# tarepan/DDSP-SVC-official

Hardware: AMD Instinct MI355X
Metric: audio samples/sec @44.1kHz CombSub synth (higher is better)
Workload: dtype f32 storage and accumulation; products of the GEMM / FIR contractions split-bf16x3 (hi*hi+hi*lo+lo*hi), of the attention split-bf16 from three pieces (6 products) for the feature projections and two (3 products) for the context sums; everything else f32; `value_fp32_mfma` is the leg with every produ; 1 GPU; CombSub 44.1 kHz, batch=64x2 s per GPU (Fr=172, T=88064), units/f0/volume/spk_id -> audio, seeded random weights, in-kernel noise

## Files before the change

ddsp-svc-official_amd/csrc/gemm_f32.h:

```cpp
#pragma once
#include "common.h"

#include <stdlib.h>
#include <type_traits>

namespace gemm {

enum { A_PLAIN = 0, A_CONV3 = 1, A_FRAMES = 2, A_CONVK = 3 };

struct Args {
    const float* A;
    const float* B;
    int M, N, K;
    int64_t lda, ldb;
    int zdiv;
    int64_t sA_hi, sA_lo, sB_hi, sB_lo;
    int Fr, Cin;
    int tap_shift;
    int ktaps, dil;
    float in_slope;
    const float* zeros;
    int sub_from, parent_tn;
    int math;
    const float* B_split;
    int A_split;
    int xcd;
    int xcd_cut;
    int kz;
};

constexpr int BK = 32;
// ... 800 lines not shown
```

ddsp-svc-official_amd/csrc/gemm_ln.h:

```cpp
#pragma once
#include "gemm_f32.h"

#include <atomic>
#include <stdlib.h>

namespace gemm {

struct LnArgs {
    const float* A;
    const float* W;
    int64_t lda, ldw;
    int M, K;
    const float* bias;
    const float* res;
    float* X;
    const float* gamma;
    const float* beta;
    float* Y;
    int y_split;
    int Fr = 1, Cin = 32, tap_shift = 0;
    const float* zeros = nullptr;
};

struct PreResidual {
    struct State {
        f32x4 res[2][4];
        f32x4 bias4[4];
    };
    template <int RB>
    __device__ __forceinline__ void load(State& s, const LnArgs& g, int m0, int rg0, int lr, int cg, int lh) const {
#pragma unroll
        for (int b = 0; b < RB; ++b) {
            const int row_m = m0 + 32 * (rg0 + b) + lr;
#pragma unroll
            for (int q = 0; q < 4; ++q) {
                s.res[b][q] = f32x4{0.f, 0.f, 0.f, 0.f};
                if (row_m < g.M) s.res[b][q] = *(const f32x4*)(g.res + (int64_t)row_m * 256 + 32 * cg + 8 * q + 4 * lh);
            }
        }
#pragma unroll
        for (int q = 0; q < 4; ++q) s.bias4[q] = *(const f32x4*)(g.bias + 32 * cg + 8 * q + 4 * lh);
    }
    __device__ __forceinline__ f32x4 apply(const State& s, const LnArgs&, int b, int q, int, int, f32x4 acc) const {
        f32x4 v;
#pragma unroll
        for (int e = 0; e < 4; ++e) v[e] = s.res[b][q][e] + (acc[e] + s.bias4[q][e]);
        return v;
    }
};

constexpr int LN_BM = 64, LN_N = 256, LN_NS = 4;
constexpr int LN_STAGE = (LN_BM + LN_N) * 32;
constexpr size_t LN_LDS_BYTES = (size_t)LN_NS * LN_STAGE * sizeof(float);

template <int NS, int RB, bool ASPLIT, int A_MODE, class Pre>
__global__ void __launch_bounds__(1024 / RB) kernel_res_ln(LnArgs g, Pre pre) {
    extern __shared__ __attribute__((aligned(1024))) float ln_lds[];
    float* const lds = ln_lds;
    constexpr int NWAVE = 16 / RB;
    const int tid = threadIdx.x, lane = tid & 63, wave = __builtin_amdgcn_readfirstlane(tid >> 6);
    const int rg0 = RB == 1 ? wave >> 3 : 0, cg = wave & 7, lr = lane & 31, lh = lane >> 5;
    const int nk = g.K / 32;
    const int m0 = blockIdx.x * LN_BM;

    typename Pre::State pst;
    pre.template load<RB>(pst, g, m0, rg0, lr, cg, lh);
    f32x4 gam4[4], bet4[4];
#pragma unroll
    for (int q = 0; q < 4; ++q) {
        const int c0 = 32 * cg + 8 * q + 4 * lh;
        gam4[q] = *(const f32x4*)(g.gamma + c0);
        bet4[q] = *(const f32x4*)(g.beta + c0);
    }

    constexpr int MAXP = RB == 1 ? 3 : 5;
    const float* src[MAXP];
    const float *src_m1 = nullptr, *src_p1 = nullptr;
#pragma unroll
    for (int i = 0; i < MAXP; ++i) {
        const int piece = wave + NWAVE * i;
        const int row = piece * 8 + (lane >> 3);
        const int slot = (lane & 7) ^ ((row >> 1) & 7);
        if (row < LN_BM) {
            int m = m0 + row;
            m = m < g.M ? m : g.M - 1;
            src[i] = g.A + (int64_t)m * g.lda + slot * 4;
            if constexpr (A_MODE == A_CONV3) {
                const int f = m % g.Fr, sh = g.tap_shift;
                const float* base = src[i];
                const float* zp = g.zeros + slot * 4;
                src_m1 = (f - 1 + sh >= 0 && f - 1 + sh < g.Fr) ? base + (int64_t)(sh - 1) * g.lda : zp;
                src_p1 = (f + 1 + sh >= 0 && f + 1 + sh < g.Fr) ? base + (int64_t)(sh + 1) * g.lda : zp;
                src[i] = (f + sh >= 0 && f + sh < g.Fr) ? base + (int64_t)sh * g.lda : zp;
            }
        } else {
            const int n = row - LN_BM < LN_N ? row - LN_BM : LN_N - 1;
            src[i] = g.W + (int64_t)n * g.ldw + slot * 4;
        }
    }
    static_assert(A_MODE == A_PLAIN || (A_MODE == A_CONV3 && RB == 2), "conv mode: eight waves, one A piece each");
    auto issue = [&](int kt) {
        float* const st = lds + (kt % NS) * LN_STAGE;
        int tap = 1, koff = kt * 32;
        if constexpr (A_MODE == A_CONV3) {
            tap = koff / g.Cin;
            koff -= tap * g.Cin;
        }
#pragma unroll
        for (int i = 0; i < MAXP; ++i)
            if (RB == 2 || i < 2 || wave < 8) {
                const float* p = src[i] + kt * 32;
                if constexpr (A_MODE == A_CONV3) {
                    if (i == 0) p = (tap == 0 ? src_m1 : tap == 1 ? src[0] : src_p1) + koff;
                }
                __builtin_amdgcn_global_load_lds((const __attribute__((address_space(1))) void*)p,
                                                 (__attribute__((address_space(3))) void*)(st + (wave + NWAVE * i) * 256), 16, 0, 0);
            }
    };
#pragma unroll
    for (int i = 0; i < NS - 1; ++i)
        if (i < nk) issue(i);

    typedef __bf16 bf16x8 __attribute__((ext_vector_type(8)));
    f32x16 acc[RB];
#pragma unroll
    for (int b = 0; b < RB; ++b)
#pragma unroll
        for (int r = 0; r < 16; ++r) acc[b][r] = 0.f;
    for (int kt = 0; kt < nk; ++kt) {
        if (kt + NS - 2 < nk) {
            if (RB == 2)
                asm volatile("s_waitcnt vmcnt(%0)" ::"n"(5 * (NS - 2)) : "memory");
            else if (wave < 8)
                asm volatile("s_waitcnt vmcnt(%0)" ::"n"(3 * (NS - 2)) : "memory");
            else
                asm volatile("s_waitcnt vmcnt(%0)" ::"n"(2 * (NS - 2)) : "memory");
        } else
            asm volatile("s_waitcnt vmcnt(0)" ::: "memory");
        __builtin_amdgcn_s_barrier();
        if (kt + NS - 1 < nk) issue(kt + NS - 1);
        const float* st = lds + (kt % NS) * LN_STAGE;
        f32x4 xv[RB][4], wv[4];
#pragma unroll
        for (int b = 0; b < RB; ++b) {
            const int row = 32 * (rg0 + b) + lr;
            const float* rp = st + row * 32;
#pragma unroll
            for (int c = 0; c < 4; ++c) xv[b][c] = *(const f32x4*)(rp + 4 * ((4 * lh + c) ^ ((row >> 1) & 7)));
        }
        {
            const int row = LN_BM + 32 * cg + lr;
            const float* rp = st + row * 32;
#pragma unroll
            for (int c = 0; c < 4; ++c) wv[c] = *(const f32x4*)(rp + 4 * ((4 * lh + c) ^ ((row >> 1) & 7)));
        }
#pragma unroll
        for (int half = 0; half < 2; ++half) {
            const bf16x8 wh = __builtin_bit_cast(bf16x8, wv[2 * half]), wl = __builtin_bit_cast(bf16x8, wv[2 * half + 1]);
#pragma unroll
            for (int b = 0; b < RB; ++b) {
                bf16x8 xh, xl;
                if constexpr (ASPLIT) {
                    xh = __builtin_bit_cast(bf16x8, xv[b][2 * half]);
                    xl = __builtin_bit_cast(bf16x8, xv[b][2 * half + 1]);
                } else {
                    typedef float f32x2p __attribute__((ext_vector_type(2)));
                    typedef __bf16 bf16x2p __attribute__((ext_vector_type(2)));
                    ddsp_u32x4 wh_, wl_;
#pragma unroll
                    for (int d = 0; d < 4; ++d) {
                        const f32x4& src = d < 2 ? xv[b][2 * half] : xv[b][2 * half + 1];
                        f32x2p r = {src[(2 * d) & 3], src[(2 * d + 1) & 3]};
                        const uint32_t hh = __builtin_bit_cast(uint32_t, __builtin_convertvector(r, bf16x2p));
                        wh_[d] = hh;
                        r = r - (f32x2p){__builtin_bit_cast(float, hh << 16), __builtin_bit_cast(float, hh & 0xffff0000u)};
                        wl_[d] = __builtin_bit_cast(uint32_t, __builtin_convertvector(r, bf16x2p));
                    }
                    xh = __builtin_bit_cast(bf16x8, wh_);
                    xl = __builtin_bit_cast(bf16x8, wl_);
                }
                acc[b] = __builtin_amdgcn_mfma_f32_32x32x16_bf16(wh, xl, acc[b], 0, 0, 0);
                acc[b] = __builtin_amdgcn_mfma_f32_32x32x16_bf16(wl, xh, acc[b], 0, 0, 0);
                acc[b] = __builtin_amdgcn_mfma_f32_32x32x16_bf16(wh, xh, acc[b], 0, 0, 0);
            }
        }
    }
    constexpr int PP = 65;
    float* const P1 = lds;
    float* const P2 = lds + LN_BM * PP;
    float* const TOT = lds + 2 * LN_BM * PP;
    __syncthreads();
    f32x4 v[RB][4];
#pragma unroll
    for (int b = 0; b < RB; ++b) {
        const int row = 32 * (rg0 + b) + lr;
#pragma unroll
        for (int q = 0; q < 4; ++q) {
            const int mr = m0 + row < g.M ? m0 + row : g.M - 1;
            v[b][q] = pre.apply(pst, g, b, q, mr, 32 * cg + 8 * q + 4 * lh,
                                f32x4{acc[b][4 * q], acc[b][4 * q + 1], acc[b][4 * q + 2], acc[b][4 * q + 3]});
            P1[row * PP + 8 * cg + 2 * q + lh] = (v[b][q][0] + v[b][q][1]) + (v[b][q][2] + v[b][q][3]);
            if (m0 + row < g.M) *(f32x4*)(g.X + (int64_t)(m0 + row) * LN_N + 32 * cg + 8 * q + 4 * lh) = v[b][q];
        }
    }
    __syncthreads();
    auto tree = [&](const float* Pm, float (&out)[RB]) {
#pragma unroll
        for (int b = 0; b < RB; ++b) {
// ... 49 lines not shown
        }
    }
}

inline bool res_ln_ok(const LnArgs& g) {
    return g.K % 32 == 0 && g.K >= 64 && g.lda % 4 == 0 && g.ldw % 4 == 0 && g.M >= 1 &&
           (((uintptr_t)g.A | (uintptr_t)g.W | (uintptr_t)g.bias | (uintptr_t)g.res | (uintptr_t)g.X | (uintptr_t)g.gamma |
             (uintptr_t)g.beta | (uintptr_t)g.Y) % 16) == 0;
}

template <int RB, bool ASPLIT, int A_MODE = A_PLAIN, class Pre = PreResidual>
inline hipError_t launch_res_ln_rb(hipStream_t st, const LnArgs& g, const Pre& pre = Pre{}) {
    static std::atomic<uint64_t> done{0};
    int dev = 0;
    hipError_t e = hipGetDevice(&dev);
    if (e != hipSuccess) return e;
    const uint64_t bit = 1ull << (dev & 63);
    auto kfn = kernel_res_ln<LN_NS, RB, ASPLIT, A_MODE, Pre>;
    if (!(done.load(std::memory_order_acquire) & bit)) {
        e = hipFuncSetAttribute((const void*)kfn, hipFuncAttributeMaxDynamicSharedMemorySize, (int)LN_LDS_BYTES);
        if (e != hipSuccess) return e;
        done.fetch_or(bit, std::memory_order_release);
    }
    hipLaunchKernelGGL(kfn, dim3((unsigned)((g.M + LN_BM - 1) / LN_BM)), dim3(1024 / RB), LN_LDS_BYTES, st, g, pre);
    return hipSuccess;
}
inline hipError_t launch_res_ln(hipStream_t st, const LnArgs& g, bool a_split = true) {
    return a_split ? launch_res_ln_rb<2, true>(st, g) : launch_res_ln_rb<2, false>(st, g);
}

}
```

ddsp-svc-official_amd/csrc/unit2ctrl_fwd.hip:

```cpp
#include "gemm_f32.h"
#include "gemm_ws.h"
#include "gemm_ln.h"
#include "performer_attn.h"
#include "u2c.h"

using namespace u2c;

namespace {

__device__ __forceinline__ void store_group8(float* __restrict__ dst, const float (&x)[8], bool split) {
    if (split) {
        ddsp_u32x4 hi, lo;
        ddsp_split8(x, hi, lo);
        *(ddsp_u32x4*)dst = hi;
        *(ddsp_u32x4*)(dst + 4) = lo;
    } else {
        *(f32x4*)dst = f32x4{x[0], x[1], x[2], x[3]};
        *(f32x4*)(dst + 4) = f32x4{x[4], x[5], x[6], x[7]};
    }
}

__device__ __forceinline__ void pack_conv3_body(const float* __restrict__ w, int Cout, int Cin, float* __restrict__ out,
                                                int vb, int vgrid, bool split) {
    const int64_t groups = (int64_t)Cout * 3 * (Cin / 8);
// ... 334 lines not shown
        return v;
    }
};

struct PreEmbed {
    EpiEmbed e;
    struct State {};
    template <int RB>
    __device__ __forceinline__ void load(State&, const gemm::LnArgs&, int, int, int, int, int) const {}
    __device__ __forceinline__ f32x4 apply(const State&, const gemm::LnArgs&, int, int, int m, int c0, f32x4 acc) const {
        return e.embed4(m, c0, acc);
    }
};

struct LnPending {
    const float* part;
    const float* bias;
    float* x_out;
    int has_res;
};
constexpr int KS_SPLITS = 4;
constexpr int KS_MAX_ROWS = 256;
constexpr int64_t U2C_PRESPLIT_MIN_ROWS = 8192;
constexpr int64_t ATTN_BF16_MIN = 256;
__global__ void __launch_bounds__(256) layernorm_kernel(const float* __restrict__ x, const float* __restrict__ gamma,
                                                        const float* __restrict__ beta, int64_t rows,
                                                        float* __restrict__ out, int split, LnPending pend = LnPending{nullptr, nullptr, nullptr, 0}) {
    const int lane = threadIdx.x & 63;
    const int64_t m = (int64_t)blockIdx.x * 4 + (threadIdx.x >> 6);
    if (m >= rows) return;
    f32x4 v;
    if (pend.part) {
        const f32x4 p0 = *(const f32x4*)(pend.part + m * D + lane * 4), p1 = *(const f32x4*)(pend.part + (rows + m) * D + lane * 4);
        const f32x4 p2 = *(const f32x4*)(pend.part + (2 * rows + m) * D + lane * 4), p3 = *(const f32x4*)(pend.part + (3 * rows + m) * D + lane * 4);
        v = (p0 + p1) + (p2 + p3);
        if (pend.bias) v = v + *(const f32x4*)(pend.bias + lane * 4);
        if (pend.has_res) v = *(const f32x4*)(x + m * D + lane * 4) + v;
        *(f32x4*)(pend.x_out + m * D + lane * 4) = v;
    } else {
        v = *(const f32x4*)(x + m * D + lane * 4);
    }
    const float mean = wave_sum((v[0] + v[1]) + (v[2] + v[3])) * (1.0f / D);
    f32x4 d;
    float ss = 0.f;
#pragma unroll
    for (int j = 0; j < 4; ++j) {
// ... 595 lines not shown
        if (fuse_glu) {
            gemm::Args g = gemm::make(b.y2, D, bf.wglu + (size_t)l * 2 * INNER * D, D, iM, 2 * INNER, D);
            set_b(g, bf.wglu + (size_t)l * 2 * INNER * D, asplit);
            EpiGlu e{b.glu, bf.bglu + (size_t)l * 2 * INNER};
            DDSP_REQUIRE(ctx, gemm::dma_ok(g) && ((uintptr_t)b.glu % 16) == 0, "unit2ctrl: fused GLU needs aligned activations");
            if (glu_large) {
                PROF(PF_U2C_GEMM_LINEAR, 2.0 * M * 2 * INNER * D, 4.0 * M * (D + INNER),
                     (gemm::dma_go<128, 128, EpiGlu, 2>(st, g, 1, e)));
            } else {
                PROF(PF_U2C_GEMM_LINEAR, 2.0 * M * 2 * INNER * D, 4.0 * M * (D + INNER),
                     (gemm::dma_go<64, 128, EpiGlu, 3, 4>(st, g, 1, e)));
            }
        } else {
            {
                gemm::Args g = gemm::make(b.y2, D, L.cm_pw1_w, D, iM, 2 * INNER, D);
                g.math = lin_math;
                gemm::EpiStore e{b.g1, 2 * INNER, L.cm_pw1_b, 1, 0, 0};
                PROF(PF_U2C_GEMM_LINEAR, 2.0 * M * 2 * INNER * D, 4.0 * M * (D + 2 * INNER),
                     (gemm::launch<true, true, gemm::A_PLAIN>(st, g, 1, e)));
            }
            PROF(PF_U2C_ROWWISE, 0, 12.0 * M * INNER,
                 hipLaunchKernelGGL(glu_kernel, dim3(grid_for(M * (INNER / 4))), dim3(256), 0, st, b.g1, M, b.glu));
        }
        PROF(PF_U2C_ROWWISE, 2.0 * M * INNER * DWK, 8.0 * M * INNER,
             if (!b.pre && dw_tiled && B * ((Fr + 15) / 16) >= 512)
                 hipLaunchKernelGGL(dwconv_tile_kernel, dim3(INNER / DWT_C, (unsigned)(B * ((Fr + DWT_F - 1) / DWT_F))), dim3(256), 0, st,
                                    b.glu, bf.wdw + (size_t)l * DWK * INNER, L.cm_dw_b, (int)B, (int)Fr, b.dwo, w.causal ? DWK - 1 : DWK / 2, asplit, in.n_frames);
             else if (!b.pre && B * ((Fr + 15) / 16) >= 512)
                 hipLaunchKernelGGL((dwconv_pair_kernel<16>), dim3(1, (unsigned)(B * ((Fr + 15) / 16))), dim3(256), 0, st,
                                    b.glu, bf.wdw + (size_t)l * DWK * INNER, L.cm_dw_b, (int)B, (int)Fr, b.dwo, w.causal ? DWK - 1 : DWK / 2, asplit, in.n_frames);
             else if (B * ((Fr + DW_RUN - 1) / DW_RUN) >= 64)
                 hipLaunchKernelGGL((dwconv_kernel<true, false>), dim3(INNER / 256, (unsigned)(B * ((Fr + DW_RUN - 1) / DW_RUN))),
                                    dim3(256), 0, st, b.glu, bf.wdw + (size_t)l * DWK * INNER, L.cm_dw_b, (int)B, (int)Fr, b.dwo, b.pre, 1, INNER, w.causal ? DWK - 1 : DWK / 2, asplit, in.n_frames);
             else
                 hipLaunchKernelGGL((dwconv_kernel<true, false, 8>), dim3(INNER / 256, (unsigned)(B * ((Fr + 7) / 8))),
                                    dim3(256), 0, st, b.glu, bf.wdw + (size_t)l * DWK * INNER, L.cm_dw_b, (int)B, (int)Fr, b.dwo, b.pre, 1, INNER, w.causal ? DWK - 1 : DWK / 2, asplit, in.n_frames));
        {
            gemm::Args g = gemm::make(b.dwo, INNER, L.cm_pw2_w, INNER, iM, D, INNER);
            set_b(g, bf.wpw2 + (size_t)l * D * INNER, asplit);
            const float* n_g = l + 1 < 3 ? w.layer[l + 1].norm_w : w.final_ln_w;
            const float* n_b = l + 1 < 3 ? w.layer[l + 1].norm_b : w.final_ln_b;
            float* n_y = l + 1 < 3 ? bf.l[l + 1].y : bf.y_final;
            const gemm::LnArgs la = ln_args(g, b.x_mid, b.x_out, L.cm_pw2_b, n_g, n_b, n_y);
            if (ln_fusable(g, la)) {
                PROF(PF_U2C_GEMM_LINEAR, 2.0 * M * D * INNER, 4.0 * M * (INNER + 4 * D), DDSP_HIP(ctx, gemm::launch_res_ln(st, la, g.A_split != 0)));
                ln_done = true;
// ... 86 lines not shown
    const bool cached = slot != nullptr;
    if (cached) {
        Arena wa{ctx, false, 0, 0};
        wa.ext = slot->dev;
        wa.ext_cap = slot->bytes;
        plan_weights(wa, bf, w);
        if (wa.rc) return wa.rc;
        bf.wstate = &slot->state;
    }
    Arena dry{ctx, true, 0, 0};
    {
        U2CBufs scratch_plan;
        plan_forward(dry, scratch_plan, w, B, Fr, false, false);
    }
    rc = ddsp_scratch_reserve_bytes(ctx, dry.total + 4096);
    if (rc) return rc;
    ddsp_scratch_reset(ctx);
    Arena a{ctx, false, 0, 0};
    plan_forward(a, bf, w, B, Fr, false, cached);
    if (a.rc) return a.rc;
    return u2c_forward(ctx, st, w, in, bf, ctrl);
}

extern "C" int ddsp_unit2ctrl_fwd(ddsp_ctx* ctx, void* stream, const ddsp_u2c_weights* wp, const float* units,
                                  const float* f0_frames, const float* phase_frames, const float* volume,
                                  const int64_t* spk_id, int64_t n_spk_id, const int64_t* mix_ids_host,
                                  const float* mix_w_host, int n_mix, int64_t B, int64_t Fr, float* ctrl) {
    return unit2ctrl_fwd_any(ctx, stream, wp, units, f0_frames, phase_frames, volume, spk_id, n_spk_id, mix_ids_host, mix_w_host,
                             n_mix, B, Fr, nullptr, ctrl);
}

extern "C" int ddsp_unit2ctrl_fwd_ragged(ddsp_ctx* ctx, void* stream, const ddsp_u2c_weights* wp, const float* units,
                                         const float* f0_frames, const float* phase_frames, const float* volume,
                                         const int64_t* spk_id, int64_t n_spk_id, const int64_t* mix_ids_host,
                                         const float* mix_w_host, int n_mix, int64_t B, int64_t Fr, const int32_t* n_frames,
                                         float* ctrl) {
    DDSP_REQUIRE(ctx, ctx && n_frames, "ddsp_unit2ctrl_fwd_ragged: null n_frames");
    return unit2ctrl_fwd_any(ctx, stream, wp, units, f0_frames, phase_frames, volume, spk_id, n_spk_id, mix_ids_host, mix_w_host,
                             n_mix, B, Fr, n_frames, ctrl);
}

static int unit2ctrl_fwd_rowmix_any(ddsp_ctx* ctx, void* stream, const ddsp_u2c_weights* wp, const float* units,
                                    const float* f0_frames, const float* phase_frames, const float* volume,
                                    const int32_t* mix_ids_dev, const float* mix_w_dev, int K, int64_t B, int64_t Fr,
                                    const int32_t* n_frames, float* ctrl) {
    DDSP_REQUIRE(ctx, ctx && mix_ids_dev && mix_w_dev, "ddsp_unit2ctrl_fwd_rowmix: null mix table");
// ... 62 lines not shown
```

ddsp-svc-official_amd/hipddsp/__init__.py:

```python
import ctypes
import numbers
import os
import threading

import torch

_HERE = os.path.dirname(os.path.abspath(__file__))
LIB_PATH = os.path.join(_HERE, "libddsp_amd.so")

DDSP_OK, DDSP_ERR_ARG, DDSP_ERR_HIP, DDSP_ERR_OOM = 0, -1, -2, -3

COMB_NONE, COMB_SINC, COMB_SINC_GATED = 0, 1, 2
FIR_ALLPASS, FIR_DYNAMIC, FIR_STATIC = 0, 1, 2
EXC_AUDIO, EXC_UNIT_NOISE, EXC_GENERATE = 0, 1, 2
FIR_FP32, FIR_SPLIT_BF16 = 0, 3
ABI_VERSION = 7
MATH_FP32, MATH_SPLIT_BF16 = 0, 3
ATTENTION_CAUSAL = 200
SLICER_PAD = {"constant": 0, "reflect": 1}
ATTENTION_PAIR = 100

_c = ctypes
_vp, _i64, _u64, _int, _f32, _f64 = _c.c_void_p, _c.c_int64, _c.c_uint64, _c.c_int, _c.c_float, _c.c_double

# ... 112 lines not shown
    "ddsp_ctx_reserve": (_int, [_vp, _u64]),
    "ddsp_ctx_poll_error": (_int, [_vp]),
    "ddsp_ctx_set_math": (_int, [_vp, _int]),
    "ddsp_ctx_get_math": (_int, [_vp]),
    "ddsp_upsample": (_int, [_vp, _vp, _vp, _i64, _i64, _i64, _int, _vp]),
    "ddsp_phase_scan": (_int, [_vp, _vp, _vp, _vp, _i64, _i64, _int, _int, _int, _int, _vp, _vp, _vp, _vp, _vp]),
    "ddsp_fir_from_ctrl": (_int, [_vp, _vp, _int, _vp, _i64, _int, _vp, _i64, _int, _vp]),
    "ddsp_ltv_fir_bwd": (_int, [_vp, _vp, _vp, _int, _u64, _vp, _vp, _i64, _i64, _int, _int, _vp, _vp]),
    "ddsp_fir_from_ctrl_bwd": (_int, [_vp, _vp, _int, _vp, _i64, _int, _vp, _i64, _int, _vp, _vp, _i64]),
    "ddsp_sins_bank": (_int, [_vp, _vp, _vp, _i64, _int, _vp, _vp, _i64, _i64, _int, _int, _vp]),
    "ddsp_spectral_ola": (_int, [_vp, _vp, _vp, _i64, _vp, _vp, _int, _u64, _i64, _i64, _int, _vp]),
    "ddsp_sins_bank_bwd": (_int, [_vp, _vp, _vp, _i64, _int, _vp, _vp, _vp, _i64, _i64, _int, _int, _vp, _i64]),
    "ddsp_spectral_ola_bwd": (_int, [_vp, _vp, _vp, _i64, _vp, _vp, _int, _u64, _vp, _i64, _i64, _int, _vp, _i64]),
    "ddsp_rss_loss": (_int, [_vp, _vp, _vp, _vp, _i64, _i64, _c.POINTER(_int), _c.POINTER(_int), _int, _f32, _f32, _vp, _vp]),
    "ddsp_sola": (_int, [_vp, _vp, _vp, _i64, _int, _int, _int, _int, _vp, _vp, _vp]),
    "ddsp_volume_gate": (_int, [_vp, _vp, _vp, _vp, _f32, _i64, _i64, _int]),
    "ddsp_volume_gate_rows": (_int, [_vp, _vp, _vp, _vp, _vp, _vp, _f32, _i64, _i64, _i64, _int]),
    "ddsp_stitch": (_int, [_vp, _vp, _vp, _i64, _vp, _i64]),
    "ddsp_phase_vocoder": (_int, [_vp, _vp, _vp, _vp, _vp, _vp, _int, _vp]),
    "ddsp_volume_extract": (_int, [_vp, _vp, _vp, _i64, _i64, _int, _vp]),
    "ddsp_volume_extract_frac": (_int, [_vp, _vp, _vp, _i64, _i64, _f64, _vp]),
    "ddsp_align_units": (_int, [_vp, _vp, _vp, _i64, _i64, _i64, _i64, _f32, _vp]),
    "ddsp_gemm_res_ln": (_int, [_vp, _vp, _vp, _vp, _vp, _vp, _vp, _vp, _int, _int, _vp, _vp, _int]),
    "ddsp_conv1d_pair_supported": (_int, [_vp, _int, _int, _int]),
    "ddsp_conv1d_pair": (_int, [_vp, _vp, _vp, _vp, _vp, _vp, _vp, _i64, _int, _int, _int, _f32, _vp, _vp]),
    "ddsp_retime_f0": (_int, [_vp, _vp, _vp, _i64, _f64, _f64, _f32, _f64, _i64, _vp]),
    "ddsp_resample_length": (_i64, [_i64, _int, _int]),
    "ddsp_resample": (_int, [_vp, _vp, _vp, _i64, _i64, _int, _int, _int, _vp]),
    "ddsp_conv1d": (_int, [_vp, _vp, _vp, _vp, _vp, _i64, _int, _int, _int, _int, _f32, _vp, _vp, _vp, _f32, _vp, _int]),
    "ddsp_nsf_source": (_int, [_vp, _vp, _vp, _vp, _vp, _vp, _i64, _int, _int, _f32, _vp]),
    "ddsp_nsf_noise_conv": (_int, [_vp, _vp, _vp, _i64, _vp, _vp, _int, _int, _int, _int, _i64, _vp]),
    "ddsp_nsf_post": (_int, [_vp, _vp, _vp, _vp, _vp, _i64, _int, _int, _f32, _vp]),
    "ddsp_nsf_mean": (_int, [_vp, _vp, _vp, _vp, _vp, _int, _i64, _vp, _vp, _f32, _int]),
    "ddsp_log_mel": (_int, [_vp, _vp, _vp, _vp, _vp, _i64, _int, _int, _f32, _vp]),
    "ddsp_adamw_step": (_int, [_vp, _vp, _vp, _vp, _vp, _vp, _i64, _f32, _f32, _f32, _f32, _f32, _i64]),
    "ddsp_adamw_step_multi": (_int, [_vp, _vp, _int, _vp, _vp, _vp, _vp, _vp, _f32, _f32, _f32, _f32, _f32, _i64]),
    "ddsp_gemm_f32": (_int, [_vp, _vp, _vp, _i64, _int, _vp, _i64, _int, _vp, _vp, _i64, _int, _int, _int, _int, _int]),
    "ddsp_performer_attention": (_int, [_vp, _vp, _vp, _vp, _vp, _vp, _i64, _i64, _vp, _int]),
    "ddsp_hubert_frames": (_i64, [_i64]),
    "ddsp_hubert_soft_units": (_int, [_vp, _vp, _c.POINTER(HubertWeights), _vp, _i64, _i64, _vp]),
    "ddsp_hubert_encode": (_int, [_vp, _vp, _c.POINTER(HubertWeights), _vp, _i64, _i64, _int, _vp]),
    "ddsp_softmax_attention": (_int, [_vp, _vp, _vp, _vp, _vp, _i64, _i64, _int, _vp, _int]),
    "ddsp_hubert_soft_units_ragged": (_int, [_vp, _vp, _c.POINTER(HubertWeights), _vp, _i64, _i64, _vp, _vp]),
    "ddsp_hubert_encode_ragged": (_int, [_vp, _vp, _c.POINTER(HubertWeights), _vp, _i64, _i64, _vp, _int, _vp]),
    "ddsp_softmax_attention_ragged": (_int, [_vp, _vp, _vp, _vp, _vp, _i64, _i64, _int, _vp, _int, _vp]),
    "ddsp_resample_ragged": (_int, [_vp, _vp, _vp, _i64, _i64, _vp, _int, _int, _int, _vp]),
# ... 636 lines not shown
        act = torch.empty(T, Cout, device=x.device, dtype=torch.float32) if act_slope is not None else None
        if out is None and act is None:
            raise ValueError("conv1d: nothing to return")
        flags = (CONV_X_SPLIT if x_split else 0) | (CONV_ACT_SPLIT if act_split else 0)
        geom = (Cin, Cout, int(ktaps), int(dil), float(in_slope), _ptr(residual), _ptr(out), _ptr(act),
                float(act_slope if act_slope is not None else 1.0), _ptr(w_split), flags)
        if rows is not None:
            B, n_dev, scale = rows
            if T % int(B):
                raise ValueError("conv1d: x must hold B rows of equal padded length")
            self.call("ddsp_conv1d_ragged", _ptr(x), _ptr(w_packed), _ptr(bias), int(B), T // int(B), *geom, _ptr(n_dev), int(scale))
        else:
            self.call("ddsp_conv1d", _ptr(x), _ptr(w_packed), _ptr(bias), T, *geom)
        return out if act_slope is None else (out, act)

    def gemm_res_ln(self, A_split, W_split, bias, res, gamma, beta, y_split=True, a_fp32=False):
        M, K = A_split.shape
        X = torch.empty(M, 256, device=A_split.device, dtype=torch.float32)
        Y = torch.empty(M, 256, device=A_split.device, dtype=torch.float32)
        self.call("ddsp_gemm_res_ln", _ptr(A_split), _ptr(W_split), _ptr(bias), _ptr(res), _ptr(gamma), _ptr(beta), int(M), int(K),
                  _ptr(X), _ptr(Y), (1 if y_split else 0) | (2 if a_fp32 else 0))
        return X, Y

    def conv1d_pair_supported(self, C, ktaps, dil):
        return bool(self.lib.ddsp_conv1d_pair_supported(self.handle, int(C), int(ktaps), int(dil)))

    def conv1d_pair(self, x, w1, b1, w2, b2, ktaps, dil, slope, want_out=True, want_act=False, rows=None):
        T, C = x.shape
        out = torch.empty(T, C, device=x.device, dtype=torch.float32) if want_out else None
        act = torch.empty(T, C, device=x.device, dtype=torch.float32) if want_act else None
        weights = (_ptr(w1), _ptr(b1), _ptr(w2), _ptr(b2))
        geom = (C, int(ktaps), int(dil), float(slope), _ptr(out), _ptr(act))
        if rows is not None:
            B, n_dev, scale = rows
            if T % int(B):
                raise ValueError("conv1d_pair: x must hold B rows of equal padded length")
            self.call("ddsp_conv1d_pair_ragged", _ptr(x), *weights, int(B), T // int(B), *geom, _ptr(n_dev), int(scale))
        else:
            self.call("ddsp_conv1d_pair", _ptr(x), *weights, T, *geom)
        return out, act

    def nsf_source(self, f0, rand_ini, lin_w, lin_b, upp, sr, sine_amp=0.1, n_dev=None):
        solo = f0.dim() == 1
        if solo and n_dev is not None:
            raise ValueError("nsf_source: n_dev needs f0 (B, L)")
        if not solo and tuple(rand_ini.shape) != (f0.shape[0], 9):
# ... 525 lines not shown
```

include/ddsp_amd.h:

```cpp
#ifndef DDSP_AMD_H
#define DDSP_AMD_H

#include <stdint.h>

#ifdef __cplusplus
extern "C" {
#endif

#define DDSP_OK 0
#define DDSP_ERR_ARG (-1)
#define DDSP_ERR_HIP (-2)
#define DDSP_ERR_OOM (-3)

typedef struct ddsp_ctx ddsp_ctx;

int ddsp_ctx_create(ddsp_ctx** out, int device);
int ddsp_ctx_destroy(ddsp_ctx* ctx);
const char* ddsp_last_error(const ddsp_ctx* ctx);
int ddsp_ctx_reserve(ddsp_ctx* ctx, uint64_t bytes);
int ddsp_abi_version(void);
int ddsp_ctx_poll_error(ddsp_ctx* ctx);
#define DDSP_MATH_FP32 0
#define DDSP_MATH_SPLIT_BF16 3
int ddsp_ctx_set_math(ddsp_ctx* ctx, int math);
// ... 243 lines not shown
int ddsp_nsf_source_ragged(ddsp_ctx* ctx, void* stream, const float* f0, const float* rand_ini, const float* lin_w,
                           const float* lin_b, int64_t B, int64_t L, int upp, int sr, float sine_amp, const int32_t* n_frames,
                           float* out);
int ddsp_nsf_noise_conv_ragged(ddsp_ctx* ctx, void* stream, const float* src, int64_t B, int64_t T_src, const float* w,
                               const float* b, int C, int K, int stride, int pad, int64_t T_out, float* out);
int ddsp_nsf_post_ragged(ddsp_ctx* ctx, void* stream, const float* x, const float* w, const float* b, int64_t B, int64_t T, int C,
                         int K, float slope, float* out, const int32_t* n_frames, int frame_scale);
int ddsp_stft_frames_ragged(ddsp_ctx* ctx, void* stream, const float* audio, int64_t B, int64_t T, const int32_t* n_samples,
                            int n_fft, int hop, int64_t L, float* out);

int ddsp_adamw_step(ddsp_ctx* ctx, void* stream, float* param, const float* grad, float* exp_avg, float* exp_avg_sq,
                    int64_t n, float lr, float beta1, float beta2, float eps, float weight_decay, int64_t step);
int ddsp_adamw_step_multi(ddsp_ctx* ctx, void* stream, int n_tensors, float* const* params, const float* const* grads,
                          float* const* exp_avg, float* const* exp_avg_sq, const int64_t* numel, float lr,
                          float beta1, float beta2, float eps, float weight_decay, int64_t step);

int ddsp_gemm_f32(ddsp_ctx* ctx, void* stream, const float* A, int64_t lda, int a_k_contig, const float* B,
                  int64_t ldb, int b_k_contig, const float* bias, float* C, int64_t ldc, int M, int N, int K, int tile,
                  int variant);

int ddsp_gemm_res_ln(ddsp_ctx* ctx, void* stream, const float* A_split, const float* W_split, const float* bias,
                     const float* res, const float* gamma, const float* beta, int M, int K, float* X, float* Y, int y_split);

#define DDSP_ATTENTION_CAUSAL 200
#define DDSP_ATTENTION_PAIR 100
int ddsp_performer_attention(ddsp_ctx* ctx, void* stream, const float* q, const float* k, const float* v,
                             const float* proj, int64_t B, int64_t Fr, float* out, int math);

typedef struct ddsp_hubert_layer {
    const float *in_proj_w, *in_proj_b, *out_proj_w, *out_proj_b, *linear1_w, *linear1_b, *linear2_w, *linear2_b;
    const float *norm1_w, *norm1_b, *norm2_w, *norm2_b;
} ddsp_hubert_layer;

typedef struct ddsp_hubert_weights {
    const float *conv0_w, *norm0_w, *norm0_b;
    const float* conv_w[6];
    const float *fp_norm_w, *fp_norm_b, *fp_proj_w, *fp_proj_b;
    const float *pos_b, *pos_g, *pos_v;
    const float *norm_w, *norm_b;
    ddsp_hubert_layer layer[12];
    const float *proj_w, *proj_b;
    uint64_t version;
} ddsp_hubert_weights;

int64_t ddsp_hubert_frames(int64_t T);
int ddsp_hubert_soft_units(ddsp_ctx* ctx, void* stream, const ddsp_hubert_weights* w, const float* wav, int64_t B, int64_t T,
// ... 78 lines not shown
```

Measured before the change: 5.075 billion samples/s.

## Fuse depthwise conv and SiLU into pointwise GEMM with residual LayerNorm

```diff
diff --git a/ddsp-svc-official_amd/csrc/gemm_f32.h b/ddsp-svc-official_amd/csrc/gemm_f32.h
--- a/ddsp-svc-official_amd/csrc/gemm_f32.h
+++ b/ddsp-svc-official_amd/csrc/gemm_f32.h
@@ -6,7 +6,7 @@
 
 namespace gemm {
 
-enum { A_PLAIN = 0, A_CONV3 = 1, A_FRAMES = 2, A_CONVK = 3 };
+enum { A_PLAIN = 0, A_CONV3 = 1, A_FRAMES = 2, A_CONVK = 3, A_DWCONV = 4 };
 
 struct Args {
     const float* A;
diff --git a/ddsp-svc-official_amd/csrc/gemm_ln.h b/ddsp-svc-official_amd/csrc/gemm_ln.h
--- a/ddsp-svc-official_amd/csrc/gemm_ln.h
+++ b/ddsp-svc-official_amd/csrc/gemm_ln.h
@@ -20,6 +20,10 @@
     int y_split;
     int Fr = 1, Cin = 32, tap_shift = 0;
     const float* zeros = nullptr;
+    const float* dw_taps = nullptr;
+    const float* dw_bias = nullptr;
+    const int* n_frames = nullptr;
+    int dw_left = 15;
 };
 
 struct PreResidual {
@@ -52,6 +56,11 @@
 constexpr int LN_BM = 64, LN_N = 256, LN_NS = 4;
 constexpr int LN_STAGE = (LN_BM + LN_N) * 32;
 constexpr size_t LN_LDS_BYTES = (size_t)LN_NS * LN_STAGE * sizeof(float);
+
+constexpr int DWF_K = 31, DWF_C = 64, DWF_ROWS = LN_BM + DWF_K - 1, DWF_NSW = 3;
+constexpr int DWF_W = LN_N * 32, DWF_IMG = LN_BM * 32;
+constexpr int DWF_AIMG = DWF_NSW * DWF_W, DWF_RAW = DWF_AIMG + 4 * DWF_IMG, DWF_TAPS = DWF_RAW + 96 * DWF_C;
+static_assert(DWF_TAPS + 32 * DWF_C == LN_NS * LN_STAGE, "the A_DWCONV layout fills the same LDS");
 
 template <int NS, int RB, bool ASPLIT, int A_MODE, class Pre>
 __global__ void __launch_bounds__(1024 / RB) kernel_res_ln(LnArgs g, Pre pre) {
@@ -61,7 +70,15 @@
     const int tid = threadIdx.x, lane = tid & 63, wave = __builtin_amdgcn_readfirstlane(tid >> 6);
     const int rg0 = RB == 1 ? wave >> 3 : 0, cg = wave & 7, lr = lane & 31, lh = lane >> 5;
     const int nk = g.K / 32;
-    const int m0 = blockIdx.x * LN_BM;
+    int m0 = blockIdx.x * LN_BM;
+    int dw_b = 0, dw_f0 = 0;
+    if constexpr (A_MODE == A_DWCONV) {
+        const int ftiles = (g.Fr + LN_BM - 1) / LN_BM;
+        dw_b = blockIdx.x / ftiles;
+        dw_f0 = (blockIdx.x % ftiles) * LN_BM;
+        m0 = dw_b * g.Fr + dw_f0;
+        g.M = dw_b * g.Fr + (dw_f0 + LN_BM < g.Fr ? dw_f0 + LN_BM : g.Fr);
+    }
 
     typename Pre::State pst;
     pre.template load<RB>(pst, g, m0, rg0, lr, cg, lh);
@@ -72,7 +89,159 @@
         gam4[q] = *(const f32x4*)(g.gamma + c0);
         bet4[q] = *(const f32x4*)(g.beta + c0);
     }
-
+    static_assert(A_MODE == A_PLAIN || ((A_MODE == A_CONV3 || A_MODE == A_DWCONV) && RB == 2), "conv modes: eight waves, one A piece each");
+    static_assert(A_MODE != A_DWCONV || ASPLIT, "the convolved operand is written in the split layout");
+
+    typedef __bf16 bf16x8 __attribute__((ext_vector_type(8)));
+    f32x16 acc[RB];
+#pragma unroll
+    for (int b = 0; b < RB; ++b)
+#pragma unroll
+        for (int r = 0; r < 16; ++r) acc[b][r] = 0.f;
+    auto products = [&](const float* ast, const float* wst) {
+        f32x4 xv[RB][4], wv[4];
+#pragma unroll
+        for (int b = 0; b < RB; ++b) {
+            const int row = 32 * (rg0 + b) + lr;
+            const float* rp = ast + row * 32;
+#pragma unroll
+            for (int c = 0; c < 4; ++c) xv[b][c] = *(const f32x4*)(rp + 4 * ((4 * lh + c) ^ ((row >> 1) & 7)));
+        }
+        {
+            const int row = 32 * cg + lr;
+            const float* rp = wst + row * 32;
+#pragma unroll
+            for (int c = 0; c < 4; ++c) wv[c] = *(const f32x4*)(rp + 4 * ((4 * lh + c) ^ ((row >> 1) & 7)));
+        }
+#pragma unroll
+        for (int half = 0; half < 2; ++half) {
+            const bf16x8 wh = __builtin_bit_cast(bf16x8, wv[2 * half]), wl = __builtin_bit_cast(bf16x8, wv[2 * half + 1]);
+#pragma unroll
+            for (int b = 0; b < RB; ++b) {
+                bf16x8 xh, xl;
+                if constexpr (ASPLIT) {
+                    xh = __builtin_bit_cast(bf16x8, xv[b][2 * half]);
+                    xl = __builtin_bit_cast(bf16x8, xv[b][2 * half + 1]);
+                } else {
+                    typedef float f32x2p __attribute__((ext_vector_type(2)));
+                    typedef __bf16 bf16x2p __attribute__((ext_vector_type(2)));
+                    ddsp_u32x4 wh_, wl_;
+#pragma unroll
+                    for (int d = 0; d < 4; ++d) {
+                        const f32x4& src = d < 2 ? xv[b][2 * half] : xv[b][2 * half + 1];
+                        f32x2p r = {src[(2 * d) & 3], src[(2 * d + 1) & 3]};
+                        const uint32_t hh = __builtin_bit_cast(uint32_t, __builtin_convertvector(r, bf16x2p));
+                        wh_[d] = hh;
+                        r = r - (f32x2p){__builtin_bit_cast(float, hh << 16), __builtin_bit_cast(float, hh & 0xffff0000u)};
+                        wl_[d] = __builtin_bit_cast(uint32_t, __builtin_convertvector(r, bf16x2p));
+                    }
+                    xh = __builtin_bit_cast(bf16x8, wh_);
+                    xl = __builtin_bit_cast(bf16x8, wl_);
+                }
+                acc[b] = __builtin_amdgcn_mfma_f32_32x32x16_bf16(wh, xl, acc[b], 0, 0, 0);
+                acc[b] = __builtin_amdgcn_mfma_f32_32x32x16_bf16(wl, xh, acc[b], 0, 0, 0);
+                acc[b] = __builtin_amdgcn_mfma_f32_32x32x16_bf16(wh, xh, acc[b], 0, 0, 0);
+            }
+        }
+    };
+
+    if constexpr (A_MODE == A_DWCONV) {
+        typedef float f32x2d __attribute__((ext_vector_type(2)));
+        typedef __bf16 bf16x2d __attribute__((ext_vector_type(2)));
+        float* const aimg = lds + DWF_AIMG;
+        float* const raw = lds + DWF_RAW;
+        float* const taps = lds + DWF_TAPS;
+        const int nb = nk / 2;
+        const int n_in = ddsp_row_frames(g.n_frames, dw_b, g.Fr);
+        const int c4 = lane & 15;
+        const float* rsrc[3];
+        int radv[3];
+#pragma unroll
+        for (int i = 0; i < 3; ++i) {
+            const int r = (wave + 8 * i) * 4 + (lane >> 4);
+            const int f = dw_f0 + r - g.dw_left;
+            const bool ok = r < DWF_ROWS && f >= 0 && f < n_in;
+            rsrc[i] = ok ? g.A + ((int64_t)dw_b * g.Fr + f) * g.lda + 4 * c4 : g.zeros + 4 * c4;
+            radv[i] = ok ? DWF_C : 0;
+        }
+        const int trow = 4 * wave + (lane >> 4);
+        const float* const tsrc = trow < DWF_K ? g.dw_taps + (int64_t)trow * g.K + 4 * c4 : g.dw_bias + 4 * c4;
+        const float* wsrc[4];
+#pragma unroll
+        for (int i = 0; i < 4; ++i) {
+            const int n = (wave + 8 * i) * 8 + (lane >> 3);
+            wsrc[i] = g.W + (int64_t)n * g.ldw + 4 * ((lane & 7) ^ ((n >> 1) & 7));
+        }
+        auto dma = [&](const float* p, float* dst) {
+            __builtin_amdgcn_global_load_lds((const __attribute__((address_space(1))) void*)p,
+                                             (__attribute__((address_space(3))) void*)dst, 16, 0, 0);
+        };
+        auto issue_raw = [&](int j) {
+#pragma unroll
+            for (int i = 0; i < 3; ++i) dma(rsrc[i] + j * radv[i], raw + (wave + 8 * i) * 256);
+            dma(tsrc + j * DWF_C, taps + wave * 256);
+        };
+        auto issue_w = [&](int kt) {
+            float* const st = lds + (kt % DWF_NSW) * DWF_W;
+#pragma unroll
+            for (int i = 0; i < 4; ++i) dma(wsrc[i] + kt * 32, st + (wave + 8 * i) * 256);
+        };
+        issue_raw(0);
+        issue_w(0);
+        issue_w(1);
+        const int cp = tid & 31, fo = 4 * (tid >> 5);
+        const int slot_hi = 2 * ((cp & 15) >> 2), q = cp & 3;
+        for (int j = 0; j < nb; ++j) {
+            asm volatile("s_waitcnt vmcnt(8)" ::: "memory");
+            __builtin_amdgcn_s_barrier();
+            {
+                const float* rw = raw + fo * DWF_C + 2 * cp;
+                const float* tp = taps + 2 * cp;
+                f32x2d win[4 + DWF_K - 1];
+#pragma unroll
+                for (int i = 0; i < 4 + DWF_K - 1; ++i) win[i] = *(const f32x2d*)(rw + i * DWF_C);
+                f32x2d a4[4];
+#pragma unroll
+                for (int o = 0; o < 4; ++o) a4[o] = *(const f32x2d*)(tp + DWF_K * DWF_C);
+#pragma unroll
+                for (int t = 0; t < DWF_K; ++t) {
+                    const f32x2d wt = *(const f32x2d*)(tp + t * DWF_C);
+#pragma unroll
+                    for (int o = 0; o < 4; ++o) a4[o] = __builtin_elementwise_fma(wt, win[o + t], a4[o]);
+                }
+                float* const img = aimg + (j & 1) * 2 * DWF_IMG + (cp >> 4) * DWF_IMG;
+#pragma unroll
+                for (int o = 0; o < 4; ++o) {
+                    f32x2d y;
+#pragma unroll
+                    for (int e = 0; e < 2; ++e)
+                        y[e] = a4[o][e] * __builtin_amdgcn_rcpf(1.0f + __builtin_amdgcn_exp2f(-1.44269504088896341f * a4[o][e]));
+                    const uint32_t h = __builtin_bit_cast(uint32_t, __builtin_convertvector(y, bf16x2d));
+                    const f32x2d rem = y - f32x2d{__builtin_bit_cast(float, h << 16), __builtin_bit_cast(float, h & 0xffff0000u)};
+                    const uint32_t l = __builtin_bit_cast(uint32_t, __builtin_convertvector(rem, bf16x2d));
+                    const int row = fo + o, sw = (row >> 1) & 7;
+                    uint32_t* const rp = (uint32_t*)(img + row * 32);
+                    rp[4 * (slot_hi ^ sw) + q] = h;
+                    rp[4 * ((slot_hi + 1) ^ sw) + q] = l;
+                }
+            }
+            __syncthreads();
+            if (j + 1 < nb) issue_raw(j + 1);
+#pragma unroll
+            for (int s = 0; s < 2; ++s) {
+                const int kt = 2 * j + s;
+                if (j + 1 < nb)
+                    asm volatile("s_waitcnt vmcnt(8)" ::: "memory");
+                else if (s == 0)
+                    asm volatile("s_waitcnt vmcnt(4)" ::: "memory");
+                else
+                    asm volatile("s_waitcnt vmcnt(0)" ::: "memory");
+                __builtin_amdgcn_s_barrier();
+                if (kt + 2 < nk) issue_w(kt + 2);
+                products(aimg + (j & 1) * 2 * DWF_IMG + s * DWF_IMG, lds + (kt % DWF_NSW) * DWF_W);
+            }
+        }
+    } else {
     constexpr int MAXP = RB == 1 ? 3 : 5;
     const float* src[MAXP];
     const float *src_m1 = nullptr, *src_p1 = nullptr;
@@ -98,7 +267,6 @@
             src[i] = g.W + (int64_t)n * g.ldw + slot * 4;
         }
     }
-    static_assert(A_MODE == A_PLAIN || (A_MODE == A_CONV3 && RB == 2), "conv mode: eight waves, one A piece each");
     auto issue = [&](int kt) {
         float* const st = lds + (kt % NS) * LN_STAGE;
         int tap = 1, koff = kt * 32;
@@ -121,12 +289,6 @@
     for (int i = 0; i < NS - 1; ++i)
         if (i < nk) issue(i);
 
-    typedef __bf16 bf16x8 __attribute__((ext_vector_type(8)));
-    f32x16 acc[RB];
-#pragma unroll
-    for (int b = 0; b < RB; ++b)
-#pragma unroll
-        for (int r = 0; r < 16; ++r) acc[b][r] = 0.f;
     for (int kt = 0; kt < nk; ++kt) {
         if (kt + NS - 2 < nk) {
             if (RB == 2)
@@ -140,50 +302,8 @@
         __builtin_amdgcn_s_barrier();
         if (kt + NS - 1 < nk) issue(kt + NS - 1);
         const float* st = lds + (kt % NS) * LN_STAGE;
-        f32x4 xv[RB][4], wv[4];
-#pragma unroll
-        for (int b = 0; b < RB; ++b) {
-            const int row = 32 * (rg0 + b) + lr;
-            const float* rp = st + row * 32;
-#pragma unroll
-            for (int c = 0; c < 4; ++c) xv[b][c] = *(const f32x4*)(rp + 4 * ((4 * lh + c) ^ ((row >> 1) & 7)));
-        }
-        {
-            const int row = LN_BM + 32 * cg + lr;
-            const float* rp = st + row * 32;
-#pragma unroll
-            for (int c = 0; c < 4; ++c) wv[c] = *(const f32x4*)(rp + 4 * ((4 * lh + c) ^ ((row >> 1) & 7)));
-        }
-#pragma unroll
-        for (int half = 0; half < 2; ++half) {
-            const bf16x8 wh = __builtin_bit_cast(bf16x8, wv[2 * half]), wl = __builtin_bit_cast(bf16x8, wv[2 * half + 1]);
-#pragma unroll
-            for (int b = 0; b < RB; ++b) {
-                bf16x8 xh, xl;
-                if constexpr (ASPLIT) {
-                    xh = __builtin_bit_cast(bf16x8, xv[b][2 * half]);
-                    xl = __builtin_bit_cast(bf16x8, xv[b][2 * half + 1]);
-                } else {
-                    typedef float f32x2p __attribute__((ext_vector_type(2)));
-                    typedef __bf16 bf16x2p __attribute__((ext_vector_type(2)));
-                    ddsp_u32x4 wh_, wl_;
-#pragma unroll
-                    for (int d = 0; d < 4; ++d) {
-                        const f32x4& src = d < 2 ? xv[b][2 * half] : xv[b][2 * half + 1];
-                        f32x2p r = {src[(2 * d) & 3], src[(2 * d + 1) & 3]};
-                        const uint32_t hh = __builtin_bit_cast(uint32_t, __builtin_convertvector(r, bf16x2p));
-                        wh_[d] = hh;
-                        r = r - (f32x2p){__builtin_bit_cast(float, hh << 16), __builtin_bit_cast(float, hh & 0xffff0000u)};
-                        wl_[d] = __builtin_bit_cast(uint32_t, __builtin_convertvector(r, bf16x2p));
-                    }
-                    xh = __builtin_bit_cast(bf16x8, wh_);
-                    xl = __builtin_bit_cast(bf16x8, wl_);
-                }
-                acc[b] = __builtin_amdgcn_mfma_f32_32x32x16_bf16(wh, xl, acc[b], 0, 0, 0);
-                acc[b] = __builtin_amdgcn_mfma_f32_32x32x16_bf16(wl, xh, acc[b], 0, 0, 0);
-                acc[b] = __builtin_amdgcn_mfma_f32_32x32x16_bf16(wh, xh, acc[b], 0, 0, 0);
-            }
-        }
+        products(st, st + LN_BM * 32);
+    }
     }
     constexpr int PP = 65;
     float* const P1 = lds;
@@ -279,11 +399,22 @@
         if (e != hipSuccess) return e;
         done.fetch_or(bit, std::memory_order_release);
     }
-    hipLaunchKernelGGL(kfn, dim3((unsigned)((g.M + LN_BM - 1) / LN_BM)), dim3(1024 / RB), LN_LDS_BYTES, st, g, pre);
+    const int64_t tiles = A_MODE == A_DWCONV ? (int64_t)(g.M / g.Fr) * ((g.Fr + LN_BM - 1) / LN_BM) : (g.M + LN_BM - 1) / LN_BM;
+    hipLaunchKernelGGL(kfn, dim3((unsigned)tiles), dim3(1024 / RB), LN_LDS_BYTES, st, g, pre);
     return hipSuccess;
 }
 inline hipError_t launch_res_ln(hipStream_t st, const LnArgs& g, bool a_split = true) {
     return a_split ? launch_res_ln_rb<2, true>(st, g) : launch_res_ln_rb<2, false>(st, g);
 }
 
-}
+inline bool res_ln_dwconv_ok(const LnArgs& g) {
+    return res_ln_ok(g) && g.K % 64 == 0 && g.Fr >= 1 && g.M % g.Fr == 0 && g.zeros && g.dw_taps && g.dw_bias && g.dw_left >= 0 &&
+           g.dw_left < DWF_K && (((uintptr_t)g.zeros | (uintptr_t)g.dw_taps | (uintptr_t)g.dw_bias) % 16) == 0;
+}
+inline bool res_ln_dwconv_fills(int64_t B, int64_t Fr) {
+    const int64_t own = B * ((Fr + LN_BM - 1) / LN_BM), rows = (B * Fr + LN_BM - 1) / LN_BM;
+    return B >= 1 && Fr >= 1 && 4 * own <= 5 * rows;
+}
+inline hipError_t launch_res_ln_dwconv(hipStream_t st, const LnArgs& g) { return launch_res_ln_rb<2, true, A_DWCONV>(st, g); }
+
+}
diff --git a/ddsp-svc-official_amd/csrc/unit2ctrl_fwd.hip b/ddsp-svc-official_amd/csrc/unit2ctrl_fwd.hip
--- a/ddsp-svc-official_amd/csrc/unit2ctrl_fwd.hip
+++ b/ddsp-svc-official_amd/csrc/unit2ctrl_fwd.hip
@@ -380,6 +380,7 @@
 constexpr int KS_SPLITS = 4;
 constexpr int KS_MAX_ROWS = 256;
 constexpr int64_t U2C_PRESPLIT_MIN_ROWS = 8192;
+constexpr int64_t U2C_DWCONV_FUSE_MIN_ROWS = 10240;
 constexpr int64_t ATTN_BF16_MIN = 256;
 __global__ void __launch_bounds__(256) layernorm_kernel(const float* __restrict__ x, const float* __restrict__ gamma,
                                                         const float* __restrict__ beta, int64_t rows,
@@ -1021,6 +1022,31 @@
             PROF(PF_U2C_ROWWISE, 0, 12.0 * M * INNER,
                  hipLaunchKernelGGL(glu_kernel, dim3(grid_for(M * (INNER / 4))), dim3(256), 0, st, b.g1, M, b.glu));
         }
+        gemm::LnArgs dwl{};
+        bool dw_fused = false;
+        {
+            gemm::Args g = gemm::make(b.glu, INNER, L.cm_pw2_w, INNER, iM, D, INNER);
+            set_b(g, bf.wpw2 + (size_t)l * D * INNER, asplit);
+            const float* n_g = l + 1 < 3 ? w.layer[l + 1].norm_w : w.final_ln_w;
+            const float* n_b = l + 1 < 3 ? w.layer[l + 1].norm_b : w.final_ln_b;
+            dwl = ln_args(g, b.x_mid, b.x_out, L.cm_pw2_b, n_g, n_b, l + 1 < 3 ? bf.l[l + 1].y : bf.y_final);
+            dwl.Fr = (int)Fr;
+            dwl.zeros = zero_page;
+            dwl.dw_taps = bf.wdw + (size_t)l * DWK * INNER;
+            dwl.dw_bias = L.cm_dw_b;
+            dwl.n_frames = in.n_frames;
+            dwl.dw_left = w.causal ? DWK - 1 : DWK / 2;
+            dw_fused = asplit && dw_tiled && M >= U2C_DWCONV_FUSE_MIN_ROWS && B * ((Fr + 15) / 16) >= 512 && ln_fusable(g, dwl) && gemm::res_ln_dwconv_ok(dwl) &&
+                       gemm::res_ln_dwconv_fills(B, Fr);
+        }
+        if (dw_fused) {
+            PROF(PF_U2C_GEMM_LINEAR, 2.0 * M * D * INNER + 2.0 * M * INNER * DWK, 4.0 * M * (INNER + 4 * D),
+                 DDSP_HIP(ctx, gemm::launch_res_ln_dwconv(st, dwl)));
+            ln_done = true;
+            ln_src = b.x_out;
+            DDSP_LAUNCH_CHECK(ctx);
+            continue;
+        }
         PROF(PF_U2C_ROWWISE, 2.0 * M * INNER * DWK, 8.0 * M * INNER,
              if (!b.pre && dw_tiled && B * ((Fr + 15) / 16) >= 512)
                  hipLaunchKernelGGL(dwconv_tile_kernel, dim3(INNER / DWT_C, (unsigned)(B * ((Fr + DWT_F - 1) / DWT_F))), dim3(256), 0, st,
@@ -1153,6 +1179,39 @@
     return u2c_forward(ctx, st, w, in, bf, ctrl);
 }
 
+extern "C" int ddsp_u2c_dwconv_pw2(ddsp_ctx* ctx, void* stream, const float* glu, const float* taps, const float* dw_bias,
+                                   const float* W_split, const float* bias, const float* res, const float* gamma,
+                                   const float* beta, const int* n_frames, int B, int Fr, int causal, int fused, float* scratch,
+                                   float* X, float* Y) {
+    DDSP_REQUIRE(ctx, ctx && glu && taps && dw_bias && W_split && bias && res && gamma && beta && X && Y && (fused || scratch),
+                 "ddsp_u2c_dwconv_pw2: null argument");
+    DDSP_REQUIRE(ctx, B >= 1 && Fr >= 1 && (int64_t)B * Fr < (1 << 26), "ddsp_u2c_dwconv_pw2: bad shape");
+    const float* zero_page = nullptr;
+    if (int rc = ddsp_zero_page(ctx, &zero_page)) return rc;
+    hipStream_t st = (hipStream_t)stream;
+    const int M = B * Fr, left = causal ? DWK - 1 : DWK / 2;
+    gemm::LnArgs a{fused ? glu : scratch, W_split, INNER, INNER, M, INNER, bias, res, X, gamma, beta, Y, 1};
+    a.Fr = Fr;
+    a.zeros = zero_page;
+    a.dw_taps = taps;
+    a.dw_bias = dw_bias;
+    a.n_frames = n_frames;
+    a.dw_left = left;
+    DDSP_REQUIRE(ctx, gemm::res_ln_dwconv_ok(a) && ((uintptr_t)glu % 16) == 0, "ddsp_u2c_dwconv_pw2: 16-byte aligned operands");
+    DDSP_ENTER_DEVICE(ctx);
+    ddsp_prof_begin(ctx, st, PF_OTHER);
+    if (fused) {
+        DDSP_HIP(ctx, gemm::launch_res_ln_dwconv(st, a));
+    } else {
+        hipLaunchKernelGGL(dwconv_tile_kernel, dim3(INNER / DWT_C, (unsigned)(B * ((Fr + DWT_F - 1) / DWT_F))), dim3(256), 0, st, glu,
+                           taps, dw_bias, B, Fr, scratch, left, 1, n_frames);
+        DDSP_HIP(ctx, gemm::launch_res_ln(st, a, true));
+    }
+    ddsp_prof_end(ctx, st, 2.0 * M * (double)D * INNER + 2.0 * M * (double)INNER * DWK, 4.0 * M * (INNER + 4.0 * D));
+    DDSP_LAUNCH_CHECK(ctx);
+    return DDSP_OK;
+}
+
 extern "C" int ddsp_unit2ctrl_fwd(ddsp_ctx* ctx, void* stream, const ddsp_u2c_weights* wp, const float* units,
                                   const float* f0_frames, const float* phase_frames, const float* volume,
                                   const int64_t* spk_id, int64_t n_spk_id, const int64_t* mix_ids_host,
diff --git a/ddsp-svc-official_amd/hipddsp/__init__.py b/ddsp-svc-official_amd/hipddsp/__init__.py
--- a/ddsp-svc-official_amd/hipddsp/__init__.py
+++ b/ddsp-svc-official_amd/hipddsp/__init__.py
@@ -158,6 +158,7 @@
     "ddsp_volume_extract_frac": (_int, [_vp, _vp, _vp, _i64, _i64, _f64, _vp]),
     "ddsp_align_units": (_int, [_vp, _vp, _vp, _i64, _i64, _i64, _i64, _f32, _vp]),
     "ddsp_gemm_res_ln": (_int, [_vp, _vp, _vp, _vp, _vp, _vp, _vp, _vp, _int, _int, _vp, _vp, _int]),
+    "ddsp_u2c_dwconv_pw2": (_int, [_vp] * 11 + [_int, _int, _int, _int, _vp, _vp, _vp]),
     "ddsp_conv1d_pair_supported": (_int, [_vp, _int, _int, _int]),
     "ddsp_conv1d_pair": (_int, [_vp, _vp, _vp, _vp, _vp, _vp, _vp, _i64, _int, _int, _int, _f32, _vp, _vp]),
     "ddsp_retime_f0": (_int, [_vp, _vp, _vp, _i64, _f64, _f64, _f32, _f64, _i64, _vp]),
@@ -840,6 +841,17 @@
                   _ptr(X), _ptr(Y), (1 if y_split else 0) | (2 if a_fp32 else 0))
         return X, Y
 
+    def u2c_dwconv_pw2(self, glu, taps, dw_bias, W_split, bias, res, gamma, beta, B, n_frames=None, causal=False, fused=True):
+        M = glu.shape[0]
+        if M % int(B):
+            raise ValueError("u2c_dwconv_pw2: glu must hold B utterances of equal padded length")
+        X = torch.empty(M, 256, device=glu.device, dtype=torch.float32)
+        Y = torch.empty(M, 256, device=glu.device, dtype=torch.float32)
+        scratch = None if fused else torch.empty(M, 512, device=glu.device, dtype=torch.float32)
+        self.call("ddsp_u2c_dwconv_pw2", _ptr(glu), _ptr(taps), _ptr(dw_bias), _ptr(W_split), _ptr(bias), _ptr(res), _ptr(gamma),
+                  _ptr(beta), _ptr(n_frames), int(B), M // int(B), 1 if causal else 0, 1 if fused else 0, _ptr(scratch), _ptr(X), _ptr(Y))
+        return X, Y
+
     def conv1d_pair_supported(self, C, ktaps, dil):
         return bool(self.lib.ddsp_conv1d_pair_supported(self.handle, int(C), int(ktaps), int(dil)))
 
diff --git a/include/ddsp_amd.h b/include/ddsp_amd.h
--- a/include/ddsp_amd.h
+++ b/include/ddsp_amd.h
@@ -289,6 +289,10 @@
 int ddsp_gemm_res_ln(ddsp_ctx* ctx, void* stream, const float* A_split, const float* W_split, const float* bias,
                      const float* res, const float* gamma, const float* beta, int M, int K, float* X, float* Y, int y_split);
 
+int ddsp_u2c_dwconv_pw2(ddsp_ctx* ctx, void* stream, const float* glu, const float* taps, const float* dw_bias,
+                        const float* W_split, const float* bias, const float* res, const float* gamma, const float* beta,
+                        const int* n_frames, int B, int Fr, int causal, int fused, float* scratch, float* X, float* Y);
+
 #define DDSP_ATTENTION_CAUSAL 200
 #define DDSP_ATTENTION_PAIR 100
 int ddsp_performer_attention(ddsp_ctx* ctx, void* stream, const float* q, const float* k, const float* v,
```

Result: faster. 5.143 billion samples/s (median of 6 runs) (+1.3%).
